# Sewer56/dxt-lossless-transform

Hardware: AMD Instinct MI355X
Metric: GiB/s BC blocks transformed (fwd+inv) (higher is better)
Workload: dtype u8

## Files before the change

### dxt-lossless-transform_amd/csrc/batch_api.cpp

```cpp
#include <hip/hip_runtime_api.h>

#include <algorithm>
#include <condition_variable>
#include <cstdlib>
#include <cstring>
#include <exception>
#include <mutex>
#include <thread>
#include <vector>

#include "../../include/dxtlt_gfx950.h"
#include "bcn_launch.h"
#include "granule_launch.h"
#include "host_common.h"

namespace {

using namespace dxtlt_host;
using dxtlt::BatchEntry;

inline uint32_t item_block_bytes(uint8_t format) { return format == 1 || format == 4 ? 8u : 16u; }

constexpr int kSlots = 4;

struct TableSlot {
    void* host = nullptr;
    void* host_mapped = nullptr;
    void* dev = nullptr;
    size_t cap = 0;
    hipEvent_t done = nullptr;
    bool pending = false;
};

struct TableRing {
    int device = -1;
    TableSlot slots[kSlots];
    int next = 0;

    ~TableRing() { release(); }
    void release()
    {
        if (device < 0)
            return;
        for (auto& s : slots) {
            if (s.host) (void)hipHostFree(s.host);
            if (s.dev) (void)hipFree(s.dev);
            if (s.done) (void)hipEventDestroy(s.done);
            s = TableSlot{};
        }
        device = -1;
        next = 0;
    }
    hipError_t acquire(size_t bytes, TableSlot** out)
    {
        int dev = 0;
        hipError_t e = hipGetDevice(&dev);
        if (e != hipSuccess)
            return e;
        if (dev != device) {
            release();
            device = dev;
        }
        TableSlot& s = slots[next];
        next = (next + 1) % kSlots;
        if (s.pending) {
            e = hipEventSynchronize(s.done);
            if (e != hipSuccess)
                return e;
            s.pending = false;
        }
        if (s.done == nullptr) {
            e = hipEventCreateWithFlags(&s.done, hipEventDisableTiming);
            if (e != hipSuccess)
                return e;
        }
        if (s.cap < bytes) {
            if (s.host) (void)hipHostFree(s.host);
            if (s.dev) (void)hipFree(s.dev);
            s.host = s.dev = nullptr;
            s.cap = 0;
            const size_t want = bytes + bytes / 2 + 4096;
            e = hipHostMalloc(&s.host, want, hipHostMallocMapped);
            if (e == hipSuccess)
                e = hipHostGetDevicePointer(&s.host_mapped, s.host, 0);
            if (e == hipSuccess)
                e = hipMalloc(&s.dev, want);
            if (e != hipSuccess)
                return e;
            s.cap = want;
        }
        *out = &s;
        return hipSuccess;
    }
};

thread_local TableRing g_ring;

const bool kTableByCopyEngine = dxtlt::experiment_env("DXTLT_BATCH_TABLE_COPY") != nullptr && dxtlt::experiment_env("DXTLT_BATCH_TABLE_COPY")[0] == '1';

hipError_t upload_table(TableSlot* slot, size_t bytes, hipStream_t stream)
{
    if (kTableByCopyEngine)
        return hipMemcpyAsync(slot->dev, slot->host, bytes, hipMemcpyHostToDevice, stream);
    return dxtlt::launch_table_upload(slot->host_mapped, slot->dev, bytes, stream);
}

}

extern "C" int32_t dxtlt_transform_batch_device(const DxtltBatchItem* items, size_t count, void* hip_stream)
{
    if (count == 0)
        return kOk;
    if (items == nullptr)
        return fail(kInvalidArgument, "NULL item array with count > 0");
    for (size_t i = 0; i < count; ++i) {
        const DxtltBatchItem& it = items[i];
        if (it.format < 1 || it.format > 7)
            return fail(kInvalidArgument, "batch item: format must be 1..5 (BC1..BC5), 6 (BC6H) or 7 (BC7; 6 and 7 are this build's "
                                          "own formats)");
        if (it.len % item_block_bytes(it.format) != 0)
            return fail(kInvalidLength, "batch item: len is not a multiple of the block size");
        if (it.decorrelation_mode > 3 && dxtlt::format_has_colour(it.format))
            return fail(kInvalidArgument, "batch item: decorrelation_mode must be 0..3");
        if (it.len > 0 && (it.d_input == nullptr || it.d_output == nullptr))
            return fail(kInvalidArgument, "batch item: NULL device buffer with len > 0");
    }
    for (const int format : {7, 6}) {
        uint64_t granules[2] = {0, 0};
        for (size_t i = 0; i < count; ++i)
            if (items[i].format == format)
                granules[items[i].inverse ? 1 : 0] += items[i].len / 16 / 1024;
        if (granules[0] > 0xFFFFFFull || granules[1] > 0xFFFFFFull)
            return fail(kInvalidArgument, dxtlt::granule::named(format, "batch too large for one launch (256 GiB or more of ", " in one direction)"));
    }
    hipStream_t user = static_cast<hipStream_t>(hip_stream);

    struct Group {
        std::vector<BatchEntry> entries;
        uint32_t wgs = 0;
        uint32_t uniform_wgs = 0;
        bool uniform = true;
    };
    constexpr int kGroups = 5 * 2 * 16;
    std::vector<Group> groups(kGroups);
    auto group_settings = [](int gi) {
        dxtlt::Settings s{};
        s.variant = (gi >> 2) & 3;
        s.split_alpha = ((gi >> 1) & 1) != 0;
        s.split_colour = (gi & 1) != 0;
        return s;
    };
    std::vector<size_t> singles;
    for (size_t i = 0; i < count; ++i) {
        const DxtltBatchItem& it = items[i];
        if (it.len == 0 || dxtlt::granule::is_granule_format(it.format))
            continue;
        if (it.len >= (size_t(64) << 30))
            return fail(kInvalidArgument, "batch item of 64 GiB or more: use the single-buffer entry point");
        const bool colour = dxtlt::format_has_colour(it.format);
        const int sa = dxtlt::format_has_alpha_split(it.format) && it.split_alpha_endpoints ? 1 : 0;
        const int sc = colour && it.split_colour_endpoints ? 1 : 0, mode = colour ? it.decorrelation_mode : 0;
        const int gi = (((it.format - 1) * 2 + (it.inverse ? 1 : 0)) << 4) | (mode << 2) | (sa << 1) | sc;
        Group& g = groups[gi];
        BatchEntry e{};
        e.src = static_cast<const uint8_t*>(it.d_input);
        e.dst = static_cast<uint8_t*>(it.d_output);
        e.blocks = it.len / item_block_bytes(it.format);
        e.first_wg = g.wgs;
        const uint32_t wgs = dxtlt::plan_batch_entry((dxtlt::Format)it.format, it.inverse != 0, group_settings(gi), e);
        if (wgs == 0xFFFFFFFFu) {
            singles.push_back(i);
            continue;
        }
        if ((uint64_t)g.wgs + wgs > 0xFFFFFFull)
            return fail(kInvalidArgument, "batch too large for one launch (64 GiB or more of one format, direction and settings)");
        g.wgs += wgs;
        g.entries.push_back(e);
        if (g.entries.size() == 1)
            g.uniform_wgs = wgs;
        else if (wgs != g.uniform_wgs)
            g.uniform = false;
    }
    static const bool no_uniform = dxtlt::experiment_env("DXTLT_BATCH_NO_UNIFORM") != nullptr;
    static const bool no_strided = dxtlt::experiment_env("DXTLT_BATCH_NO_STRIDED") != nullptr;

    using GranuleEntry = dxtlt::granule::BatchEntry;
    struct GranulePlan {
        std::vector<GranuleEntry> entries, tails;
        std::vector<uint32_t> coarse;
        uint64_t wgs = 0;
        size_t at = 0, entry_bytes = 0, tail_bytes = 0, bytes = 0;
    };
    GranulePlan granule_plans[4];
    size_t table_bytes = 0;
    for (int q = 0; q < 4; ++q) {
        GranulePlan& p = granule_plans[q];
        const int inverse = q & 1, format = q < 2 ? 7 : 6;
        for (size_t i = 0; i < count; ++i) {
            const DxtltBatchItem& it = items[i];
            if (it.format != format || it.len == 0 || (it.inverse != 0) != (inverse != 0))
                continue;
            const uint64_t blocks = it.len / 16, tail = blocks % 1024, main = blocks - tail;
            const uint8_t* src = static_cast<const uint8_t*>(it.d_input);
            uint8_t* dst = static_cast<uint8_t*>(it.d_output);
            if (main != 0) {
                p.entries.push_back({src, dst, main, (uint32_t)p.wgs, 0});
                p.wgs += main / 1024;
            }
            if (tail != 0)
                p.tails.push_back({src + main * 16, dst + main * 16, 0, 0, (uint32_t)tail});
        }
        if (p.entries.empty() && p.tails.empty())
            continue;
        p.coarse.resize(((size_t)p.wgs + 63) / 64);
        size_t cur = 0;
        for (size_t k = 0; k < p.coarse.size(); ++k) {
            while (cur + 1 < p.entries.size() && p.entries[cur + 1].first_wg <= (uint32_t)(k * 64))
                ++cur;
            p.coarse[k] = (uint32_t)cur;
        }
        p.entry_bytes = p.entries.size() * sizeof(GranuleEntry);
        p.tail_bytes = p.tails.size() * sizeof(GranuleEntry);
        p.bytes = (p.entry_bytes + p.tail_bytes + p.coarse.size() * sizeof(uint32_t) + 15) & ~(size_t)15;
        p.at = table_bytes;
        table_bytes += p.bytes;
    }

    struct Placed {
        int gi;
        size_t at, entry_bytes;
    };
    std::vector<Placed> placed;
    for (int gi = 0; gi < kGroups; ++gi) {
        const Group& g = groups[gi];
        if (g.entries.empty())
            continue;
        const size_t entry_bytes = (g.entries.size() * sizeof(BatchEntry) + 15) & ~(size_t)15;
        placed.push_back({gi, table_bytes, entry_bytes});
        table_bytes += entry_bytes + dxtlt::batch_index_bytes(g.wgs);
    }
    if (table_bytes != 0) {
        TableSlot* slot = nullptr;
        hipError_t e = g_ring.acquire(table_bytes, &slot);
        if (e != hipSuccess)
            return fail(kDevice, "batch table staging", e);
        for (const GranulePlan& p : granule_plans) {
            if (p.bytes == 0)
                continue;
            uint8_t* h = static_cast<uint8_t*>(slot->host) + p.at;
            if (p.entry_bytes) std::memcpy(h, p.entries.data(), p.entry_bytes);
            if (p.tail_bytes) std::memcpy(h + p.entry_bytes, p.tails.data(), p.tail_bytes);
            if (!p.coarse.empty()) std::memcpy(h + p.entry_bytes + p.tail_bytes, p.coarse.data(), p.coarse.size() * sizeof(uint32_t));
        }
        std::vector<bool> wide(placed.size());
        for (size_t k = 0; k < placed.size(); ++k) {
            const Group& g = groups[placed[k].gi];
            uint8_t* h = static_cast<uint8_t*>(slot->host) + placed[k].at;
            std::memcpy(h, g.entries.data(), g.entries.size() * sizeof(BatchEntry));
            wide[k] = dxtlt::build_batch_index(g.entries.data(), g.entries.size(), g.wgs, h + placed[k].entry_bytes);
        }
        e = upload_table(slot, table_bytes, user);
        const char* what = "batch table copy / launch";
        for (int q = 0; q < 4 && e == hipSuccess; ++q) {
            const GranulePlan& p = granule_plans[q];
            const int inverse = q & 1, format = q < 2 ? 7 : 6;
            if (p.bytes == 0)
                continue;
            const uint8_t* d = static_cast<const uint8_t*>(slot->dev) + p.at;
            e = dxtlt::granule::launch_batch(format, inverse != 0, reinterpret_cast<const GranuleEntry*>(d),
                                             reinterpret_cast<const uint32_t*>(d + p.entry_bytes + p.tail_bytes), (uint32_t)p.entries.size(),
                                             (uint32_t)p.wgs, reinterpret_cast<const GranuleEntry*>(d + p.entry_bytes),
                                             (uint32_t)p.tails.size(), user);
            if (e != hipSuccess)
                what = format == 7 ? "BC7 batch table copy / launch" : "BC6H batch table copy / launch";
        }
        for (size_t k = 0; k < placed.size() && e == hipSuccess; ++k) {
            const int gi = placed[k].gi;
            Group& g = groups[gi];
            const size_t n = g.entries.size();
            const bool uniform = g.uniform && !no_uniform;
            bool strided = uniform && !no_strided;
            const int64_t src_stride = n >= 2 ? (int64_t)(g.entries[1].src - g.entries[0].src) : 0;
            const int64_t dst_stride = n >= 2 ? (int64_t)(g.entries[1].dst - g.entries[0].dst) : 0;
            for (size_t i = 1; i < n && strided; ++i) {
                const BatchEntry &a = g.entries[0], &b = g.entries[i];
                strided = b.blocks == a.blocks && b.full_tiles == a.full_tiles && b.form == a.form && b.halo_vecs == a.halo_vecs &&
                          std::memcmp(b.shift, a.shift, sizeof a.shift) == 0 && std::memcmp(b.gbase, a.gbase, sizeof a.gbase) == 0 &&
                          b.src == a.src + (int64_t)i * src_stride && b.dst == a.dst + (int64_t)i * dst_stride;
            }
            const uint8_t* d = static_cast<const uint8_t*>(slot->dev) + placed[k].at;
            e = dxtlt::launch_batch((dxtlt::Format)((gi >> 5) + 1), ((gi >> 4) & 1) != 0, group_settings(gi),
                                    reinterpret_cast<const BatchEntry*>(d), d + placed[k].entry_bytes, (uint32_t)n, g.wgs,
                                    uniform ? g.uniform_wgs : 0, wide[k], user, strided ? &g.entries[0] : nullptr, src_stride, dst_stride);
        }
        hipError_t ev = hipEventRecord(slot->done, user);
        slot->pending = ev == hipSuccess;
        if (e != hipSuccess)
            return fail(kDevice, what, e);
        if (ev != hipSuccess)
            return fail(kDevice, "batch event", ev);
    }
    for (size_t i : singles) {
        const DxtltBatchItem& it = items[i];
        dxtlt::Settings s{};
        s.variant = it.decorrelation_mode;
        s.split_alpha = it.split_alpha_endpoints != 0;
        s.split_colour = it.split_colour_endpoints != 0;
        s = dxtlt::effective_settings((dxtlt::Format)it.format, s);
        const uint64_t blocks = it.len / item_block_bytes(it.format);
        const hipError_t e = dxtlt::launch_transform((dxtlt::Format)it.format, it.inverse != 0, s, it.d_input, it.d_output,
                                                     dxtlt::Range{blocks, 0, blocks}, user);
        if (e != hipSuccess)
            return fail(kDevice, "batch item launch", e);
    }
    return kOk;
}

extern "C" uint32_t dxtlt_debug_plan_batch(int32_t format, int32_t inverse, int32_t variant, int32_t split_alpha, int32_t split_colour,
                                           const uint64_t* src_addresses, const uint64_t* dst_addresses, const uint64_t* blocks, size_t count,
                                           DxtltDebugPlannedEntry* entries_out, uint8_t* index_out, size_t index_capacity,
                                           uint32_t* index_is_wide_out)
{
    if (index_is_wide_out)
        *index_is_wide_out = 0;
    if (format < 1 || format > 5 || (count != 0 && (!src_addresses || !dst_addresses || !blocks || !entries_out)))
        return 0xFFFFFFFFu;
    dxtlt::Settings s{};
    s.variant = variant;
    s.split_alpha = split_alpha != 0;
    s.split_colour = split_colour != 0;
    s = dxtlt::effective_settings((dxtlt::Format)format, s);
    std::vector<BatchEntry> entries;
    uint32_t total = 0;
    for (size_t i = 0; i < count; ++i) {
        BatchEntry e{};
        e.src = reinterpret_cast<const uint8_t*>(static_cast<uintptr_t>(src_addresses[i]));
        e.dst = reinterpret_cast<uint8_t*>(static_cast<uintptr_t>(dst_addresses[i]));
        e.blocks = blocks[i];
        e.first_wg = total;
        const uint32_t wgs = dxtlt::plan_batch_entry((dxtlt::Format)format, inverse != 0, s, e);
        if (wgs == 0xFFFFFFFFu || (uint64_t)total + wgs > 0xFFFFFFull)
            return 0xFFFFFFFFu;
        if (wgs == 0)
            e.end_wg = e.first_wg;
        total += wgs;
        DxtltDebugPlannedEntry& o = entries_out[i];
        o.first_wg = e.first_wg;
        o.end_wg = e.end_wg;
        o.full_tiles = e.full_tiles;
        o.form = e.form;
        o.halo_vecs = e.halo_vecs;
        std::memcpy(o.shift, e.shift, sizeof o.shift);
        std::memcpy(o.gbase, e.gbase, sizeof o.gbase);
        if (wgs != 0)
            entries.push_back(e);
    }
    if (total != 0) {
        if (index_out == nullptr || index_capacity < dxtlt::batch_index_bytes(total))
            return 0xFFFFFFFFu;
        const bool wide = dxtlt::build_batch_index(entries.data(), entries.size(), total, index_out);
        if (index_is_wide_out)
            *index_is_wide_out = wide ? 1 : 0;
    }
    return total;
}

// ... 353 lines not shown
```

### dxt-lossless-transform_amd/csrc/batch_kernels.hip

```cpp
#include <cstdlib>
#include <cstring>
#include <vector>

#include "bcn_device.h"

namespace dxtlt {

struct BatchView {
    const uint8_t* src;
    uint8_t* dst;
    uint64_t blocks;
    uint32_t first_wg, end_wg, full_tiles;
    uint32_t flags;
    uint32_t shifts[2];
    uint64_t gbase[6];
};

__device__ __forceinline__ BatchView load_batch_entry(const BatchEntry* entry)
{
    const uint64_t* q = reinterpret_cast<const uint64_t*>(entry);
    const uint32_t* w = reinterpret_cast<const uint32_t*>(entry);
    BatchView v;
    v.src = (const uint8_t*)(global_cptr)q[0];
    v.dst = (uint8_t*)(global_ptr)q[1];
// ... 127 lines not shown
            en = load_batch_entry(entries + e);
        }
    }
    const uint32_t n_wgs = en.end_wg - en.first_wg;
    uint32_t local = wg - en.first_wg;
    if (n_wgs >= 8) {
        local += (en.first_wg + n_wgs - 1u - e) & 7u;
        local = local >= n_wgs ? local - n_wgs : local;
    }
    const bool aligned = (en.flags & 0xFF) == kBatchAligned;
    if (aligned && local < en.full_tiles) {
        if constexpr (INVERSE)
            inv_aligned_tile<FMT, VARIANT, SA, SC, THREADS>(en.src, en.dst, en.blocks, 0, local, lds);
        else
            fwd_aligned_tile<FMT, VARIANT, SA, SC, THREADS>(en.src, en.dst, en.blocks, 0, local, lds);
        WG_TIMING_END(1);
        return;
    }
    Shifts sh;
#pragma unroll
    for (int i = 0; i < 6; ++i) {
        sh.d[i] = (int)((en.shifts[i >> 2] >> (8 * (i & 3))) & 127u);
        sh.gbase[i] = en.gbase[i];
    }
#ifdef DXTLT_EXPERIMENTS
    sh.xcd_remap = 0;
    sh.line_policy = INVERSE ? 1 : 3;
    sh.skip_partial = 0;
#endif
    sh.natural = 1;
    sh.halo_vecs = (int)(en.flags >> 8) & 0xFF;
    sh.full_tiles = en.full_tiles;
    sh.range_blocks = en.blocks;
    if constexpr (INVERSE) {
        if (local < en.full_tiles) {
            const uint64_t tile = xcd_contiguous_tile(local, en.full_tiles);
            inv_shift_tile<FMT, VARIANT, SA, SC, THREADS>(en.src, en.dst, en.blocks, 0, sh, tile, lds);
            WG_TIMING_END(2);
            return;
        }
        inv_shift_edge_tile<FMT, VARIANT, SA, SC, THREADS>(en.src, en.dst, en.blocks, sh, en.full_tiles, lds);
        WG_TIMING_END(4);
    } else {
        if (local != 0 && local < en.full_tiles) {
            fwd_halo_tile<FMT, VARIANT, SA, SC, kNormNone, true, THREADS>(en.src, en.dst, en.blocks, 0, sh, local, lds);
            WG_TIMING_END(2);
            return;
        }
        fwd_halo_edge_tile<FMT, VARIANT, SA, SC, kNormNone, true, THREADS>(en.src, en.dst, sh, local, lds);
        WG_TIMING_END(local == 0 ? 3 : 4);
    }
}

uint32_t plan_batch_entry(Format fmt, bool inverse, const Settings& s, BatchEntry& e)
{
    if (e.blocks == 0)
        return 0;
    const Settings es = effective_settings(fmt, s);
    const Streams S = make_streams(fmt, es.split_alpha, es.split_colour);
    const void* soa = inverse ? (const void*)e.src : (const void*)e.dst;
    const uint64_t T = (uint64_t)tile_blocks(fmt, batch_tile_threads(fmt, es.split_colour, inverse));
    const uint64_t tiles = e.blocks / T, rest = e.blocks % T;
    const uint64_t mask = inverse ? 15 : (uint64_t)(kHaloAlign - 1);
    bool on_lines = true, stream_tails = false;
    int d[6] = {0, 0, 0, 0, 0, 0}, halo_blocks = 0;
    for (int i = 0; i < S.n; ++i) {
        const uint64_t base = reinterpret_cast<uintptr_t>(soa) + (uint64_t)S.off[i] * e.blocks;
        d[i] = (int)(base & mask);
        on_lines = on_lines && (base & 127) == 0;
        stream_tails = stream_tails || d[i] != 0;
        halo_blocks = std::max(halo_blocks, (d[i] + S.width[i] - 1) / S.width[i]);
    }
    if (!shifts_are_natural(S, d))
        return 0xFFFFFFFFu;
    e.form = on_lines ? 1 : 0;
    e.natural = 1;
    e.reserved = 0;
    e.reserved2[0] = e.reserved2[1] = 0;
    const int per_vec = 16 / fmt_block(fmt);
    e.halo_vecs = inverse ? 0 : (uint8_t)((halo_blocks + per_vec - 1) / per_vec);
    for (int i = 0; i < 6; ++i) {
        e.shift[i] = (uint8_t)d[i];
        e.gbase[i] = i < S.n ? (uint64_t)S.off[i] * e.blocks - (uint64_t)d[i] : 0;
    }
    e.full_tiles = (uint32_t)tiles;
    const bool edge = rest != 0 || (!inverse && stream_tails);
    const uint32_t wgs = (uint32_t)tiles + (edge ? 1u : 0u);
    e.end_wg = e.first_wg + wgs;
    return wgs;
}

bool build_batch_index(const BatchEntry* entries, size_t n_entries, uint32_t total_wgs, uint8_t* index)
{
    const size_t n_base = batch_index_base_count(total_wgs), n_delta = batch_index_delta_count(total_wgs);
    uint32_t* base = reinterpret_cast<uint32_t*>(index);
    std::memset(index, 0, batch_index_bytes(total_wgs));
    std::vector<uint32_t> d(n_delta);
    uint32_t largest = 0;
    size_t cur = 0;
    for (size_t j = 0; j < n_delta; ++j) {
        const uint32_t wg = (uint32_t)(j * kBatchIndexWgs);
        while (cur + 1 < n_entries && entries[cur].end_wg <= wg)
            ++cur;
        if (wg % kBatchBaseWgs == 0)
            base[wg / kBatchBaseWgs] = (uint32_t)cur;
        d[j] = (uint32_t)(cur - base[wg / kBatchBaseWgs]);
        largest = std::max(largest, d[j]);
    }
    const bool wide = largest > 255;
    uint8_t* delta = index + n_base * 4;
    for (size_t j = 0; j < n_delta; ++j) {
        if (wide) {
            delta[2 * j] = (uint8_t)d[j];
            delta[2 * j + 1] = (uint8_t)(d[j] >> 8);
        } else {
            delta[j] = (uint8_t)d[j];
        }
    }
    return wide;
}

namespace {

using BatchFn = void (*)(const BatchEntry*, const uint8_t*, uint32_t, uint32_t, uint32_t, StridedBatch);

template <int FMT, int VARIANT, bool SA, bool SC>
BatchFn batch_fn(bool inverse) { return inverse ? batch_kernel<FMT, VARIANT, SA, SC, true> : batch_kernel<FMT, VARIANT, SA, SC, false>; }

template <int FMT, int VARIANT>
BatchFn batch_splits(bool sa, bool sc, bool inverse)
{
    if constexpr (FMT == kBc3) {
        if (sa)
            return sc ? batch_fn<FMT, VARIANT, true, true>(inverse) : batch_fn<FMT, VARIANT, true, false>(inverse);
    }
    return sc ? batch_fn<FMT, VARIANT, false, true>(inverse) : batch_fn<FMT, VARIANT, false, false>(inverse);
}

template <int FMT>
BatchFn batch_bc45(bool split_endpoints, bool inverse)
{
    return split_endpoints ? batch_fn<FMT, kNone, true, false>(inverse) : batch_fn<FMT, kNone, false, false>(inverse);
}

template <int FMT>
BatchFn batch_variant(int variant, bool sa, bool sc, bool inverse)
{
    switch (variant) {
    case kNone: return batch_splits<FMT, kNone>(sa, sc, inverse);
    case kVar1: return batch_splits<FMT, kVar1>(sa, sc, inverse);
    case kVar2: return batch_splits<FMT, kVar2>(sa, sc, inverse);
    default: return batch_splits<FMT, kVar3>(sa, sc, inverse);
    }
}

}

hipError_t launch_batch(Format fmt, bool inverse, const Settings& s, const BatchEntry* d_entries, const uint8_t* d_index,
                        uint32_t n_entries, uint32_t total_wgs, uint32_t uniform_wgs, bool wide_index, hipStream_t stream,
                        const BatchEntry* strided_first, int64_t src_stride, int64_t dst_stride)
{
    if (n_entries == 0 || total_wgs == 0)
        return hipSuccess;
    if (s.variant < 0 || s.variant > 3 || total_wgs > 0xFFFFFFu)
        return hipErrorInvalidValue;
    if (uniform_wgs != 0 && (uint64_t)uniform_wgs * n_entries != total_wgs)
        return hipErrorInvalidValue;
    const uint32_t magic = uniform_wgs > 1 ? (uint32_t)((1ull << 32) / uniform_wgs) : uniform_wgs == 1 ? 0xFFFFFFFFu : n_entries;
    static const bool no_array = experiment_env("DXTLT_BATCH_NO_ARRAY") != nullptr;
    if (strided_first != nullptr && uniform_wgs != 0 && !no_array && strided_first->form == 1) {
        const hipError_t e = launch_tiled_array(fmt, inverse, s, strided_first->src, strided_first->dst, strided_first->blocks, n_entries,
// ... 29 lines not shown
```

### dxt-lossless-transform_amd/csrc/bcn_launch.h

```cpp
#pragma once
#include <hip/hip_runtime_api.h>
#include <stddef.h>
#include <stdint.h>

#include <cstdlib>

namespace dxtlt {

inline const char* experiment_env(const char* name)
{
#ifdef DXTLT_EXPERIMENTS
    return std::getenv(name);
#else
    (void)name;
    return nullptr;
#endif
}

enum Format : int { kBc1 = 1, kBc2 = 2, kBc3 = 3, kBc4 = 4, kBc5 = 5 };

struct Settings {
    int variant;
    bool split_alpha;
    bool split_colour;
// ... 106 lines not shown
    if (!format_has_colour(f)) {
        e.variant = 0;
        e.split_colour = false;
    }
    return e;
}

struct Streams {
    int n;
    int width[6];
    int off[6];
};

constexpr Streams make_streams(int fmt, bool split_alpha, bool split_colour)
{
    Streams s{};
    int n = 0, off = 0;
    if (fmt == kBc4 || fmt == kBc5) {
        for (int h = 0; h < (fmt == kBc5 ? 2 : 1); ++h) {
            if (split_alpha) {
                s.width[n] = 1; s.off[n] = off; off += 1; ++n;
                s.width[n] = 1; s.off[n] = off; off += 1; ++n;
            } else {
                s.width[n] = 2; s.off[n] = off; off += 2; ++n;
            }
            s.width[n] = 6; s.off[n] = off; off += 6; ++n;
        }
        s.n = n;
        return s;
    }
    if (fmt == kBc3) {
        if (split_alpha) {
            s.width[n] = 1; s.off[n] = off; off += 1; ++n;
            s.width[n] = 1; s.off[n] = off; off += 1; ++n;
        } else {
            s.width[n] = 2; s.off[n] = off; off += 2; ++n;
        }
        s.width[n] = 6; s.off[n] = off; off += 6; ++n;
    }
    if (fmt == kBc2) {
        s.width[n] = 8; s.off[n] = off; off += 8; ++n;
    }
    if (split_colour) {
        s.width[n] = 2; s.off[n] = off; off += 2; ++n;
        s.width[n] = 2; s.off[n] = off; off += 2; ++n;
    } else {
        s.width[n] = 4; s.off[n] = off; off += 4; ++n;
    }
    s.width[n] = 4; s.off[n] = off; off += 4; ++n;
    s.n = n;
    return s;
}

}
```

### include/dxtlt_gfx950.h

```cpp
#ifndef DXTLT_GFX950_H
#define DXTLT_GFX950_H

#include <stdbool.h>
#include <stddef.h>
#include <stdint.h>

#include "dlt_size_estimator.h"

#ifdef __cplusplus
extern "C" {
#endif

#define DXTLT_OK 0
#define DXTLT_E_INVALID_LENGTH 1
#define DXTLT_E_INVALID_ARGUMENT 2
#define DXTLT_E_NO_DEVICE 3
#define DXTLT_E_DEVICE 4
#define DXTLT_E_ESTIMATOR 5
#define DXTLT_E_ALLOCATION 6

#define DXTLT_YCOCG_NONE 0
#define DXTLT_YCOCG_VARIANT1 1
#define DXTLT_YCOCG_VARIANT2 2
#define DXTLT_YCOCG_VARIANT3 3
// ... 29 lines not shown
void dxtlt_set_auto_estimator_threads(int32_t threads);
int32_t dxtlt_get_auto_estimator_threads(void);
int32_t dxtlt_set_auto_estimator_threads_for_this_thread(int32_t cap);

int32_t dxtlt_transform_bc1_with_settings_device(const void *d_input, void *d_output, size_t len,
                                                 uint8_t decorrelation_mode, bool split_colour_endpoints,
                                                 void *hip_stream);
int32_t dxtlt_untransform_bc1_with_settings_device(const void *d_input, void *d_output, size_t len,
                                                   uint8_t decorrelation_mode, bool split_colour_endpoints,
                                                   void *hip_stream);
int32_t dxtlt_transform_bc2_with_settings_device(const void *d_input, void *d_output, size_t len,
                                                 uint8_t decorrelation_mode, bool split_colour_endpoints,
                                                 void *hip_stream);
int32_t dxtlt_untransform_bc2_with_settings_device(const void *d_input, void *d_output, size_t len,
                                                   uint8_t decorrelation_mode, bool split_colour_endpoints,
                                                   void *hip_stream);
int32_t dxtlt_transform_bc3_with_settings_device(const void *d_input, void *d_output, size_t len,
                                                 uint8_t decorrelation_mode, bool split_alpha_endpoints,
                                                 bool split_colour_endpoints, void *hip_stream);
int32_t dxtlt_untransform_bc3_with_settings_device(const void *d_input, void *d_output, size_t len,
                                                   uint8_t decorrelation_mode, bool split_alpha_endpoints,
                                                   bool split_colour_endpoints, void *hip_stream);

int32_t dxtlt_transform_range_device(int32_t format, bool inverse, const void *d_src, void *d_dst,
                                     uint64_t total_blocks, uint64_t first_block, uint64_t num_blocks,
                                     uint8_t decorrelation_mode, bool split_alpha_endpoints,
                                     bool split_colour_endpoints, void *hip_stream);

typedef struct DxtltBatchItem {
    const void *d_input;
    void *d_output;
    uint64_t len;
    uint8_t format;
    uint8_t inverse;
    uint8_t decorrelation_mode;
    uint8_t split_alpha_endpoints;
    uint8_t split_colour_endpoints;
    uint8_t reserved[3];
} DxtltBatchItem;
int32_t dxtlt_transform_batch_device(const DxtltBatchItem *items, size_t count, void *hip_stream);
typedef struct DxtltDebugPlannedEntry {
    uint32_t first_wg, end_wg;
    uint32_t full_tiles;
    uint8_t form;
    uint8_t halo_vecs;
    uint8_t shift[6];
    uint64_t gbase[6];
} DxtltDebugPlannedEntry;
uint32_t dxtlt_debug_plan_batch(int32_t format, int32_t inverse, int32_t variant, int32_t split_alpha, int32_t split_colour,
                                const uint64_t *src_addresses, const uint64_t *dst_addresses, const uint64_t *blocks, size_t count,
                                DxtltDebugPlannedEntry *entries_out, uint8_t *index_out, size_t index_capacity,
                                uint32_t *index_is_wide_out);

typedef struct DxtltDebugPlannedLaunch {
    int32_t kind;
    int32_t threads;
    uint32_t workgroups;
    uint32_t full_tiles;
    uint64_t range_blocks;
    uint64_t aos_offset;
    uint8_t shift[6];
    uint8_t halo_vecs;
    uint8_t natural;
    uint64_t gbase[6];
} DxtltDebugPlannedLaunch;
int32_t dxtlt_debug_plan_transform(int32_t format, int32_t inverse, int32_t variant, int32_t split_alpha, int32_t split_colour,
                                   uint64_t src_address, uint64_t dst_address, uint64_t total_blocks, uint64_t first_block,
                                   uint64_t num_blocks, DxtltDebugPlannedLaunch *out, int32_t cap);

int32_t dxtlt_transform_batch_host(const DxtltBatchItem *items, size_t count);

int32_t dxtlt_transform_sharded(int32_t format, bool inverse, const uint8_t *input_ptr, uint8_t *output_ptr,
                                size_t len, uint8_t decorrelation_mode, bool split_alpha_endpoints,
                                bool split_colour_endpoints, int32_t num_devices);

typedef struct DxtltShardStat {
    int32_t device;
    int32_t cpus_bound;
    uint64_t first_block;
    uint64_t blocks;
    double seconds;
} DxtltShardStat;
int32_t dxtlt_sharded_last_stats(DxtltShardStat *out, int32_t cap);

int32_t dxtlt_pci_local_cpulist(const char *pci_bdf, char *out, size_t cap);
int32_t dxtlt_device_local_cpulist(int32_t device, char *out, size_t cap);
int32_t dxtlt_bind_thread_to_cpulist(const char *cpulist);

int32_t dxtlt_fill_splitmix64_device(void *d_dst, size_t len_bytes, uint64_t seed, uint64_t first_qword,
                                     void *hip_stream);
const char *dxtlt_last_error(void);
int32_t dxtlt_device_count(void);
size_t dxtlt_host_route_threshold_bytes(void);
void dxtlt_set_host_route_threshold_bytes(size_t bytes);
void dxtlt_set_tuning(int32_t tile_threads, int32_t force_path);
int32_t dxtlt_tuning_mask(void);
const char *dxtlt_version(void);
void dxtlt_release_thread_resources(void);

#ifdef __cplusplus
}
#endif
#endif
```

Measured before the change: 3191.

## Restructure batch planning into count and place passes, skip tables for regular groups

Batch planning is split into a counting pass that builds a per-group context once and reuses the workgroup count for entries with matching size and alignment, plus a staging pass that writes entries straight into pinned host memory. Groups whose items are evenly strided with identical plans skip the per-entry table and index upload entirely and go down an array-style launch. The index builder also writes deltas in place instead of using a temporary vector. The intent is to cut host-side per-call planning, allocation and table upload costs for large batches, at the price of more complex two-pass logic that has to stay consistent between the passes.

```diff
diff --git a/dxt-lossless-transform_amd/csrc/batch_api.cpp b/dxt-lossless-transform_amd/csrc/batch_api.cpp
--- a/dxt-lossless-transform_amd/csrc/batch_api.cpp
+++ b/dxt-lossless-transform_amd/csrc/batch_api.cpp
@@ -2,6 +2,7 @@
 
 #include <algorithm>
 #include <condition_variable>
+#include <cstdio>
 #include <cstdlib>
 #include <cstring>
 #include <exception>
@@ -105,14 +106,74 @@
     return dxtlt::launch_table_upload(slot->host_mapped, slot->dev, bytes, stream);
 }
 
-}
-
-extern "C" int32_t dxtlt_transform_batch_device(const DxtltBatchItem* items, size_t count, void* hip_stream)
-{
-    if (count == 0)
-        return kOk;
-    if (items == nullptr)
-        return fail(kInvalidArgument, "NULL item array with count > 0");
+constexpr int kGroups = 5 * 2 * 16;
+
+inline dxtlt::Settings group_settings(int gi)
+{
+    dxtlt::Settings s{};
+    s.variant = (gi >> 2) & 3;
+    s.split_alpha = ((gi >> 1) & 1) != 0;
+    s.split_colour = (gi & 1) != 0;
+    return s;
+}
+
+inline int group_of(const DxtltBatchItem& it)
+{
+    const bool colour = dxtlt::format_has_colour(it.format);
+    const int sa = dxtlt::format_has_alpha_split(it.format) && it.split_alpha_endpoints ? 1 : 0;
+    const int sc = colour && it.split_colour_endpoints ? 1 : 0, mode = colour ? it.decorrelation_mode : 0;
+    return (((it.format - 1) * 2 + (it.inverse ? 1 : 0)) << 4) | (mode << 2) | (sa << 1) | sc;
+}
+
+inline uint64_t address_of(const void* p) { return static_cast<uint64_t>(reinterpret_cast<uintptr_t>(p)); }
+
+struct GroupPlan {
+    int gi = 0;
+    dxtlt::BatchGroupContext ctx{};
+    uint32_t count = 0;
+    uint32_t wgs = 0;
+    uint32_t uniform_wgs = 0;
+    bool uniform = true;
+    bool regular = true;
+    bool has_table = false;
+    bool wide = false;
+    uint64_t src0 = 0, dst0 = 0, blocks0 = 0;
+    int64_t src_stride = 0, dst_stride = 0;
+    BatchEntry first{};
+    size_t at = 0, entry_bytes = 0, index_bytes = 0;
+    uint32_t placed = 0, next_wg = 0;
+};
+
+using GranuleEntry = dxtlt::granule::BatchEntry;
+struct GranulePlan {
+    std::vector<GranuleEntry> entries, tails;
+    std::vector<uint32_t> coarse;
+    uint64_t wgs = 0;
+    size_t at = 0, entry_bytes = 0, tail_bytes = 0, bytes = 0;
+};
+
+struct BatchCallPlan {
+    std::vector<GroupPlan> groups;
+    int16_t slot_of[kGroups];
+    GranulePlan granule[4];
+    std::vector<size_t> singles;
+    size_t table_bytes = 0;
+};
+
+const bool kNoUniform = dxtlt::experiment_env("DXTLT_BATCH_NO_UNIFORM") != nullptr;
+const bool kNoStrided = dxtlt::experiment_env("DXTLT_BATCH_NO_STRIDED") != nullptr;
+const bool kNoArray = dxtlt::experiment_env("DXTLT_BATCH_NO_ARRAY") != nullptr;
+
+inline bool same_plan(const BatchEntry& a, const BatchEntry& b)
+{
+    return b.blocks == a.blocks && b.end_wg - b.first_wg == a.end_wg - a.first_wg && b.full_tiles == a.full_tiles && b.form == a.form &&
+           b.halo_vecs == a.halo_vecs && std::memcmp(b.shift, a.shift, sizeof a.shift) == 0 && std::memcmp(b.gbase, a.gbase, sizeof a.gbase) == 0;
+}
+
+int32_t plan_batch_call(const DxtltBatchItem* items, size_t count, BatchCallPlan& plan)
+{
+    uint64_t granules[4] = {0, 0, 0, 0};
+    size_t granule_items = 0;
     for (size_t i = 0; i < count; ++i) {
         const DxtltBatchItem& it = items[i];
         if (it.format < 1 || it.format > 7)
@@ -124,77 +185,70 @@
             return fail(kInvalidArgument, "batch item: decorrelation_mode must be 0..3");
         if (it.len > 0 && (it.d_input == nullptr || it.d_output == nullptr))
             return fail(kInvalidArgument, "batch item: NULL device buffer with len > 0");
-    }
-    for (const int format : {7, 6}) {
-        uint64_t granules[2] = {0, 0};
-        for (size_t i = 0; i < count; ++i)
-            if (items[i].format == format)
-                granules[items[i].inverse ? 1 : 0] += items[i].len / 16 / 1024;
-        if (granules[0] > 0xFFFFFFull || granules[1] > 0xFFFFFFull)
-            return fail(kInvalidArgument, dxtlt::granule::named(format, "batch too large for one launch (256 GiB or more of ", " in one direction)"));
-    }
-    hipStream_t user = static_cast<hipStream_t>(hip_stream);
-
-    struct Group {
-        std::vector<BatchEntry> entries;
-        uint32_t wgs = 0;
-        uint32_t uniform_wgs = 0;
-        bool uniform = true;
-    };
-    constexpr int kGroups = 5 * 2 * 16;
-    std::vector<Group> groups(kGroups);
-    auto group_settings = [](int gi) {
-        dxtlt::Settings s{};
-        s.variant = (gi >> 2) & 3;
-        s.split_alpha = ((gi >> 1) & 1) != 0;
-        s.split_colour = (gi & 1) != 0;
-        return s;
-    };
-    std::vector<size_t> singles;
+        if (dxtlt::granule::is_granule_format(it.format) && it.len != 0) {
+            granules[(it.format == 7 ? 0 : 2) + (it.inverse ? 1 : 0)] += it.len / 16 / 1024;
+            ++granule_items;
+        }
+    }
+    for (int q = 0; q < 4; ++q)
+        if (granules[q] > 0xFFFFFFull)
+            return fail(kInvalidArgument, dxtlt::granule::named(q < 2 ? 7 : 6, "batch too large for one launch (256 GiB or more of ", " in one direction)"));
+
+    std::memset(plan.slot_of, 0xFF, sizeof plan.slot_of);
     for (size_t i = 0; i < count; ++i) {
         const DxtltBatchItem& it = items[i];
         if (it.len == 0 || dxtlt::granule::is_granule_format(it.format))
             continue;
         if (it.len >= (size_t(64) << 30))
             return fail(kInvalidArgument, "batch item of 64 GiB or more: use the single-buffer entry point");
-        const bool colour = dxtlt::format_has_colour(it.format);
-        const int sa = dxtlt::format_has_alpha_split(it.format) && it.split_alpha_endpoints ? 1 : 0;
-        const int sc = colour && it.split_colour_endpoints ? 1 : 0, mode = colour ? it.decorrelation_mode : 0;
-        const int gi = (((it.format - 1) * 2 + (it.inverse ? 1 : 0)) << 4) | (mode << 2) | (sa << 1) | sc;
-        Group& g = groups[gi];
-        BatchEntry e{};
-        e.src = static_cast<const uint8_t*>(it.d_input);
-        e.dst = static_cast<uint8_t*>(it.d_output);
-        e.blocks = it.len / item_block_bytes(it.format);
-        e.first_wg = g.wgs;
-        const uint32_t wgs = dxtlt::plan_batch_entry((dxtlt::Format)it.format, it.inverse != 0, group_settings(gi), e);
+        const int gi = group_of(it);
+        if (plan.slot_of[gi] < 0) {
+            plan.slot_of[gi] = (int16_t)plan.groups.size();
+            plan.groups.emplace_back();
+            plan.groups.back().gi = gi;
+            plan.groups.back().ctx = dxtlt::make_batch_group((dxtlt::Format)it.format, it.inverse != 0, group_settings(gi));
+        }
+        GroupPlan& g = plan.groups[(size_t)plan.slot_of[gi]];
+        const uint64_t src = address_of(it.d_input), dst = address_of(it.d_output), blocks = it.len / item_block_bytes(it.format);
+        const uint64_t soa = it.inverse ? src : dst;
+        const uint32_t wgs = g.count != 0 && blocks == g.blocks0 && ((soa ^ (it.inverse ? g.src0 : g.dst0)) & 127) == 0
+                                 ? g.uniform_wgs : dxtlt::count_batch_entry(g.ctx, soa, blocks);
         if (wgs == 0xFFFFFFFFu) {
-            singles.push_back(i);
-            continue;
-        }
-        if ((uint64_t)g.wgs + wgs > 0xFFFFFFull)
-            return fail(kInvalidArgument, "batch too large for one launch (64 GiB or more of one format, direction and settings)");
+            plan.singles.push_back(i);
+            continue;
+        }
+        if ((uint64_t)g.wgs + wgs > 0xFFFFFFull) {
+            thread_local char text[160];
+            std::snprintf(text, sizeof text, "batch too large for one launch (more than 2^24 tiles of %d KiB of one format, direction and settings)",
+                          g.ctx.threads * 16 / 1024);
+            return fail(kInvalidArgument, text);
+        }
+        if (g.count == 0) {
+            g.src0 = src;
+            g.dst0 = dst;
+            g.blocks0 = blocks;
+            g.uniform_wgs = wgs;
+        } else {
+            if (g.count == 1) {
+                g.src_stride = (int64_t)(src - g.src0);
+                g.dst_stride = (int64_t)(dst - g.dst0);
+            }
+            g.uniform = g.uniform && wgs == g.uniform_wgs;
+            g.regular = g.regular && blocks == g.blocks0 && src == g.src0 + (uint64_t)g.count * (uint64_t)g.src_stride &&
+                        dst == g.dst0 + (uint64_t)g.count * (uint64_t)g.dst_stride;
+        }
         g.wgs += wgs;
-        g.entries.push_back(e);
-        if (g.entries.size() == 1)
-            g.uniform_wgs = wgs;
-        else if (wgs != g.uniform_wgs)
-            g.uniform = false;
-    }
-    static const bool no_uniform = dxtlt::experiment_env("DXTLT_BATCH_NO_UNIFORM") != nullptr;
-    static const bool no_strided = dxtlt::experiment_env("DXTLT_BATCH_NO_STRIDED") != nullptr;
-
-    using GranuleEntry = dxtlt::granule::BatchEntry;
-    struct GranulePlan {
-        std::vector<GranuleEntry> entries, tails;
-        std::vector<uint32_t> coarse;
-        uint64_t wgs = 0;
-        size_t at = 0, entry_bytes = 0, tail_bytes = 0, bytes = 0;
-    };
-    GranulePlan granule_plans[4];
-    size_t table_bytes = 0;
-    for (int q = 0; q < 4; ++q) {
-        GranulePlan& p = granule_plans[q];
+        ++g.count;
+    }
+    plan.groups.erase(std::remove_if(plan.groups.begin(), plan.groups.end(), [](const GroupPlan& g) { return g.count == 0; }), plan.groups.end());
+    std::sort(plan.groups.begin(), plan.groups.end(), [](const GroupPlan& a, const GroupPlan& b) { return a.gi < b.gi; });
+    std::memset(plan.slot_of, 0xFF, sizeof plan.slot_of);
+    for (size_t k = 0; k < plan.groups.size(); ++k)
+        plan.slot_of[plan.groups[k].gi] = (int16_t)k;
+
+    plan.table_bytes = 0;
+    for (int q = 0; q < 4 && granule_items != 0; ++q) {
+        GranulePlan& p = plan.granule[q];
         const int inverse = q & 1, format = q < 2 ? 7 : 6;
         for (size_t i = 0; i < count; ++i) {
             const DxtltBatchItem& it = items[i];
@@ -222,85 +276,139 @@
         p.entry_bytes = p.entries.size() * sizeof(GranuleEntry);
         p.tail_bytes = p.tails.size() * sizeof(GranuleEntry);
         p.bytes = (p.entry_bytes + p.tail_bytes + p.coarse.size() * sizeof(uint32_t) + 15) & ~(size_t)15;
-        p.at = table_bytes;
-        table_bytes += p.bytes;
-    }
-
-    struct Placed {
-        int gi;
-        size_t at, entry_bytes;
-    };
-    std::vector<Placed> placed;
-    for (int gi = 0; gi < kGroups; ++gi) {
-        const Group& g = groups[gi];
-        if (g.entries.empty())
-            continue;
-        const size_t entry_bytes = (g.entries.size() * sizeof(BatchEntry) + 15) & ~(size_t)15;
-        placed.push_back({gi, table_bytes, entry_bytes});
-        table_bytes += entry_bytes + dxtlt::batch_index_bytes(g.wgs);
-    }
-    if (table_bytes != 0) {
-        TableSlot* slot = nullptr;
-        hipError_t e = g_ring.acquire(table_bytes, &slot);
+        p.at = plan.table_bytes;
+        plan.table_bytes += p.bytes;
+    }
+
+    for (GroupPlan& g : plan.groups) {
+        g.first.src = reinterpret_cast<const uint8_t*>(static_cast<uintptr_t>(g.src0));
+        g.first.dst = reinterpret_cast<uint8_t*>(static_cast<uintptr_t>(g.dst0));
+        g.first.blocks = g.blocks0;
+        g.first.first_wg = 0;
+        (void)dxtlt::plan_batch_entry(g.ctx, g.first);
+        g.uniform = g.uniform && !kNoUniform;
+        g.regular = g.regular && g.uniform && !kNoStrided;
+        const int64_t soa_stride = g.ctx.inverse ? g.src_stride : g.dst_stride;
+        if (g.regular && g.count >= 2 && (soa_stride & 127) != 0) {
+            const uint32_t low = (uint32_t)(soa_stride & 127), period = 128u / (low & (0u - low));
+            for (uint32_t i = 1; i < period && i < g.count && g.regular; ++i) {
+                BatchEntry e{};
+                e.src = reinterpret_cast<const uint8_t*>(static_cast<uintptr_t>(g.src0 + (uint64_t)i * (uint64_t)g.src_stride));
+                e.dst = reinterpret_cast<uint8_t*>(static_cast<uintptr_t>(g.dst0 + (uint64_t)i * (uint64_t)g.dst_stride));
+                e.blocks = g.blocks0;
+                g.regular = dxtlt::plan_batch_entry(g.ctx, e) != 0xFFFFFFFFu && same_plan(g.first, e);
+            }
+        }
+        g.has_table = !g.regular || kNoArray;
+        if (g.has_table) {
+            g.entry_bytes = ((size_t)g.count * sizeof(BatchEntry) + 15) & ~(size_t)15;
+            g.index_bytes = dxtlt::batch_index_bytes(g.wgs);
+            g.at = plan.table_bytes;
+            plan.table_bytes += g.entry_bytes + g.index_bytes;
+        }
+    }
+    return kOk;
+}
+
+int32_t stage_batch_call(const DxtltBatchItem* items, size_t count, BatchCallPlan& plan, uint8_t* host)
+{
+    for (const GranulePlan& p : plan.granule) {
+        if (p.bytes == 0)
+            continue;
+        uint8_t* h = host + p.at;
+        if (p.entry_bytes) std::memcpy(h, p.entries.data(), p.entry_bytes);
+        if (p.tail_bytes) std::memcpy(h + p.entry_bytes, p.tails.data(), p.tail_bytes);
+        if (!p.coarse.empty()) std::memcpy(h + p.entry_bytes + p.tail_bytes, p.coarse.data(), p.coarse.size() * sizeof(uint32_t));
+    }
+    bool any = false;
+    for (const GroupPlan& g : plan.groups)
+        any = any || g.has_table;
+    if (!any)
+        return kOk;
+    for (size_t i = 0; i < count; ++i) {
+        const DxtltBatchItem& it = items[i];
+        if (it.len == 0 || dxtlt::granule::is_granule_format(it.format))
+            continue;
+        const int slot = plan.slot_of[group_of(it)];
+        if (slot < 0 || !plan.groups[(size_t)slot].has_table)
+            continue;
+        GroupPlan& g = plan.groups[(size_t)slot];
+        BatchEntry e{};
+        e.src = static_cast<const uint8_t*>(it.d_input);
+        e.dst = static_cast<uint8_t*>(it.d_output);
+        e.blocks = it.len / item_block_bytes(it.format);
+        e.first_wg = g.next_wg;
+        const uint32_t wgs = dxtlt::plan_batch_entry(g.ctx, e);
+        if (wgs == 0xFFFFFFFFu)
+            continue;
+        if (g.placed >= g.count || (uint64_t)g.next_wg + wgs > g.wgs)
+            return fail(kDevice, "batch table: the placing pass disagrees with the count pass");
+        reinterpret_cast<BatchEntry*>(host + g.at)[g.placed++] = e;
+        g.next_wg += wgs;
+    }
+    for (GroupPlan& g : plan.groups) {
+        if (!g.has_table)
+            continue;
+        if (g.placed != g.count || g.next_wg != g.wgs)
+            return fail(kDevice, "batch table: the placing pass disagrees with the count pass");
+        g.wide = dxtlt::build_batch_index(reinterpret_cast<const BatchEntry*>(host + g.at), g.count, g.wgs, host + g.at + g.entry_bytes);
+    }
+    return kOk;
+}
+
+}
+
+extern "C" int32_t dxtlt_transform_batch_device(const DxtltBatchItem* items, size_t count, void* hip_stream)
+{
+    if (count == 0)
+        return kOk;
+    if (items == nullptr)
+        return fail(kInvalidArgument, "NULL item array with count > 0");
+    BatchCallPlan plan;
+    if (const int32_t rc = plan_batch_call(items, count, plan); rc != kOk)
+        return rc;
+    hipStream_t user = static_cast<hipStream_t>(hip_stream);
+
+    TableSlot* slot = nullptr;
+    hipError_t e = hipSuccess;
+    const char* what = "batch table copy / launch";
+    if (plan.table_bytes != 0) {
+        e = g_ring.acquire(plan.table_bytes, &slot);
         if (e != hipSuccess)
             return fail(kDevice, "batch table staging", e);
-        for (const GranulePlan& p : granule_plans) {
-            if (p.bytes == 0)
-                continue;
-            uint8_t* h = static_cast<uint8_t*>(slot->host) + p.at;
-            if (p.entry_bytes) std::memcpy(h, p.entries.data(), p.entry_bytes);
-            if (p.tail_bytes) std::memcpy(h + p.entry_bytes, p.tails.data(), p.tail_bytes);
-            if (!p.coarse.empty()) std::memcpy(h + p.entry_bytes + p.tail_bytes, p.coarse.data(), p.coarse.size() * sizeof(uint32_t));
-        }
-        std::vector<bool> wide(placed.size());
-        for (size_t k = 0; k < placed.size(); ++k) {
-            const Group& g = groups[placed[k].gi];
-            uint8_t* h = static_cast<uint8_t*>(slot->host) + placed[k].at;
-            std::memcpy(h, g.entries.data(), g.entries.size() * sizeof(BatchEntry));
-            wide[k] = dxtlt::build_batch_index(g.entries.data(), g.entries.size(), g.wgs, h + placed[k].entry_bytes);
-        }
-        e = upload_table(slot, table_bytes, user);
-        const char* what = "batch table copy / launch";
-        for (int q = 0; q < 4 && e == hipSuccess; ++q) {
-            const GranulePlan& p = granule_plans[q];
-            const int inverse = q & 1, format = q < 2 ? 7 : 6;
-            if (p.bytes == 0)
-                continue;
-            const uint8_t* d = static_cast<const uint8_t*>(slot->dev) + p.at;
-            e = dxtlt::granule::launch_batch(format, inverse != 0, reinterpret_cast<const GranuleEntry*>(d),
-                                             reinterpret_cast<const uint32_t*>(d + p.entry_bytes + p.tail_bytes), (uint32_t)p.entries.size(),
-                                             (uint32_t)p.wgs, reinterpret_cast<const GranuleEntry*>(d + p.entry_bytes),
-                                             (uint32_t)p.tails.size(), user);
-            if (e != hipSuccess)
-                what = format == 7 ? "BC7 batch table copy / launch" : "BC6H batch table copy / launch";
-        }
-        for (size_t k = 0; k < placed.size() && e == hipSuccess; ++k) {
-            const int gi = placed[k].gi;
-            Group& g = groups[gi];
-            const size_t n = g.entries.size();
-            const bool uniform = g.uniform && !no_uniform;
-            bool strided = uniform && !no_strided;
-            const int64_t src_stride = n >= 2 ? (int64_t)(g.entries[1].src - g.entries[0].src) : 0;
-            const int64_t dst_stride = n >= 2 ? (int64_t)(g.entries[1].dst - g.entries[0].dst) : 0;
-            for (size_t i = 1; i < n && strided; ++i) {
-                const BatchEntry &a = g.entries[0], &b = g.entries[i];
-                strided = b.blocks == a.blocks && b.full_tiles == a.full_tiles && b.form == a.form && b.halo_vecs == a.halo_vecs &&
-                          std::memcmp(b.shift, a.shift, sizeof a.shift) == 0 && std::memcmp(b.gbase, a.gbase, sizeof a.gbase) == 0 &&
-                          b.src == a.src + (int64_t)i * src_stride && b.dst == a.dst + (int64_t)i * dst_stride;
-            }
-            const uint8_t* d = static_cast<const uint8_t*>(slot->dev) + placed[k].at;
-            e = dxtlt::launch_batch((dxtlt::Format)((gi >> 5) + 1), ((gi >> 4) & 1) != 0, group_settings(gi),
-                                    reinterpret_cast<const BatchEntry*>(d), d + placed[k].entry_bytes, (uint32_t)n, g.wgs,
-                                    uniform ? g.uniform_wgs : 0, wide[k], user, strided ? &g.entries[0] : nullptr, src_stride, dst_stride);
-        }
-        hipError_t ev = hipEventRecord(slot->done, user);
+        if (const int32_t rc = stage_batch_call(items, count, plan, static_cast<uint8_t*>(slot->host)); rc != kOk)
+            return rc;
+        e = upload_table(slot, plan.table_bytes, user);
+    }
+    for (int q = 0; q < 4 && e == hipSuccess; ++q) {
+        const GranulePlan& p = plan.granule[q];
+        const int inverse = q & 1, format = q < 2 ? 7 : 6;
+        if (p.bytes == 0)
+            continue;
+        const uint8_t* d = static_cast<const uint8_t*>(slot->dev) + p.at;
+        e = dxtlt::granule::launch_batch(format, inverse != 0, reinterpret_cast<const GranuleEntry*>(d),
+                                         reinterpret_cast<const uint32_t*>(d + p.entry_bytes + p.tail_bytes), (uint32_t)p.entries.size(),
+                                         (uint32_t)p.wgs, reinterpret_cast<const GranuleEntry*>(d + p.entry_bytes),
+                                         (uint32_t)p.tails.size(), user);
+        if (e != hipSuccess)
+            what = format == 7 ? "BC7 batch table copy / launch" : "BC6H batch table copy / launch";
+    }
+    for (size_t k = 0; k < plan.groups.size() && e == hipSuccess; ++k) {
+        const GroupPlan& g = plan.groups[k];
+        const uint8_t* d = g.has_table ? static_cast<const uint8_t*>(slot->dev) + g.at : nullptr;
+        e = dxtlt::launch_batch((dxtlt::Format)((g.gi >> 5) + 1), ((g.gi >> 4) & 1) != 0, group_settings(g.gi),
+                                reinterpret_cast<const BatchEntry*>(d), g.has_table ? d + g.entry_bytes : nullptr, g.count, g.wgs,
+                                g.uniform ? g.uniform_wgs : 0, g.wide, user, g.regular ? &g.first : nullptr, g.src_stride, g.dst_stride);
+    }
+    if (slot != nullptr) {
+        const hipError_t ev = hipEventRecord(slot->done, user);
         slot->pending = ev == hipSuccess;
-        if (e != hipSuccess)
-            return fail(kDevice, what, e);
-        if (ev != hipSuccess)
+        if (e == hipSuccess && ev != hipSuccess)
             return fail(kDevice, "batch event", ev);
     }
-    for (size_t i : singles) {
+    if (e != hipSuccess)
+        return fail(kDevice, what, e);
+    for (size_t i : plan.singles) {
         const DxtltBatchItem& it = items[i];
         dxtlt::Settings s{};
         s.variant = it.decorrelation_mode;
@@ -308,10 +416,55 @@
         s.split_colour = it.split_colour_endpoints != 0;
         s = dxtlt::effective_settings((dxtlt::Format)it.format, s);
         const uint64_t blocks = it.len / item_block_bytes(it.format);
-        const hipError_t e = dxtlt::launch_transform((dxtlt::Format)it.format, it.inverse != 0, s, it.d_input, it.d_output,
-                                                     dxtlt::Range{blocks, 0, blocks}, user);
+        e = dxtlt::launch_transform((dxtlt::Format)it.format, it.inverse != 0, s, it.d_input, it.d_output,
+                                    dxtlt::Range{blocks, 0, blocks}, user);
         if (e != hipSuccess)
             return fail(kDevice, "batch item launch", e);
+    }
+    return kOk;
+}
+
+extern "C" int32_t dxtlt_debug_plan_batch_call(const DxtltBatchItem* items, size_t count, void* staging, size_t staging_capacity,
+                                               DxtltDebugBatchCallReport* report, DxtltDebugBatchCallGroup* groups_out, size_t groups_capacity)
+{
+    if (report == nullptr || (count != 0 && items == nullptr) || (groups_capacity != 0 && groups_out == nullptr))
+        return fail(kInvalidArgument, "dxtlt_debug_plan_batch_call: NULL argument");
+    *report = DxtltDebugBatchCallReport{};
+    BatchCallPlan plan;
+    if (const int32_t rc = plan_batch_call(items, count, plan); rc != kOk)
+        return rc;
+    report->table_bytes = plan.table_bytes;
+    report->groups = (uint32_t)plan.groups.size();
+    report->singles = (uint32_t)plan.singles.size();
+    for (int q = 0; q < 4; ++q) {
+        report->granule_table_offset[q] = plan.granule[q].at;
+        report->granule_table_bytes[q] = plan.granule[q].bytes;
+    }
+    if (staging != nullptr) {
+        if (staging_capacity < plan.table_bytes || (reinterpret_cast<uintptr_t>(staging) & 15) != 0)
+            return fail(kInvalidArgument, "dxtlt_debug_plan_batch_call: the staging buffer is too small or not 16-byte aligned");
+        if (const int32_t rc = stage_batch_call(items, count, plan, static_cast<uint8_t*>(staging)); rc != kOk)
+            return rc;
+        report->staged = 1;
+    }
+    for (size_t k = 0; k < plan.groups.size() && k < groups_capacity; ++k) {
+        const GroupPlan& g = plan.groups[k];
+        const dxtlt::Settings s = group_settings(g.gi);
+        DxtltDebugBatchCallGroup& o = groups_out[k];
+        o = DxtltDebugBatchCallGroup{};
+        o.format = (uint8_t)((g.gi >> 5) + 1);
+        o.inverse = (uint8_t)((g.gi >> 4) & 1);
+        o.decorrelation_mode = (uint8_t)s.variant;
+        o.split_alpha_endpoints = s.split_alpha ? 1 : 0;
+        o.split_colour_endpoints = s.split_colour ? 1 : 0;
+        o.regular = g.regular ? 1 : 0;
+        o.wide_index = g.wide ? 1 : 0;
+        o.uniform = g.uniform ? 1 : 0;
+        o.entries = g.count;
+        o.workgroups = g.wgs;
+        o.table_offset = g.has_table ? g.at : 0;
+        o.entry_bytes = g.has_table ? g.entry_bytes : 0;
+        o.table_bytes = g.has_table ? g.entry_bytes + g.index_bytes : 0;
     }
     return kOk;
 }
diff --git a/dxt-lossless-transform_amd/csrc/batch_kernels.hip b/dxt-lossless-transform_amd/csrc/batch_kernels.hip
--- a/dxt-lossless-transform_amd/csrc/batch_kernels.hip
+++ b/dxt-lossless-transform_amd/csrc/batch_kernels.hip
@@ -203,50 +203,96 @@
     }
 }
 
-uint32_t plan_batch_entry(Format fmt, bool inverse, const Settings& s, BatchEntry& e)
+BatchGroupContext make_batch_group(Format fmt, bool inverse, const Settings& s)
+{
+    const Settings es = effective_settings(fmt, s);
+    BatchGroupContext g{};
+    g.fmt = fmt;
+    g.inverse = inverse;
+    g.threads = batch_tile_threads(fmt, es.split_colour, inverse);
+    g.tile_blocks = (uint64_t)tile_blocks(fmt, g.threads);
+    g.shift_mask = inverse ? 15 : (uint64_t)(kHaloAlign - 1);
+    g.vec_blocks = 16 / fmt_block(fmt);
+    g.streams = make_streams(fmt, es.split_alpha, es.split_colour);
+    return g;
+}
+
+namespace {
+
+inline bool batch_entry_shifts(const BatchGroupContext& g, uint64_t soa, uint64_t blocks, int (&d)[6], bool& on_lines, bool& stream_tails)
+{
+    const Streams& S = g.streams;
+    on_lines = true;
+    stream_tails = false;
+    for (int i = 0; i < 6; ++i)
+        d[i] = 0;
+    for (int i = 0; i < S.n; ++i) {
+        const uint64_t base = soa + (uint64_t)S.off[i] * blocks;
+        d[i] = (int)(base & g.shift_mask);
+        on_lines = on_lines && (base & 127) == 0;
+        stream_tails = stream_tails || d[i] != 0;
+    }
+    return shifts_are_natural(S, d) != 0;
+}
+
+inline uint32_t batch_entry_wgs(const BatchGroupContext& g, uint64_t blocks, bool stream_tails)
+{
+    const uint64_t tiles = blocks / g.tile_blocks, rest = blocks % g.tile_blocks;
+    const bool edge = rest != 0 || (!g.inverse && stream_tails);
+    return (uint32_t)tiles + (edge ? 1u : 0u);
+}
+
+}
+
+uint32_t count_batch_entry(const BatchGroupContext& g, uint64_t soa_address, uint64_t blocks)
+{
+    if (blocks == 0)
+        return 0;
+    int d[6];
+    bool on_lines, stream_tails;
+    if (!batch_entry_shifts(g, soa_address, blocks, d, on_lines, stream_tails))
+        return 0xFFFFFFFFu;
+    return batch_entry_wgs(g, blocks, stream_tails);
+}
+
+uint32_t plan_batch_entry(const BatchGroupContext& g, BatchEntry& e)
 {
     if (e.blocks == 0)
         return 0;
-    const Settings es = effective_settings(fmt, s);
-    const Streams S = make_streams(fmt, es.split_alpha, es.split_colour);
-    const void* soa = inverse ? (const void*)e.src : (const void*)e.dst;
-    const uint64_t T = (uint64_t)tile_blocks(fmt, batch_tile_threads(fmt, es.split_colour, inverse));
-    const uint64_t tiles = e.blocks / T, rest = e.blocks % T;
-    const uint64_t mask = inverse ? 15 : (uint64_t)(kHaloAlign - 1);
-    bool on_lines = true, stream_tails = false;
-    int d[6] = {0, 0, 0, 0, 0, 0}, halo_blocks = 0;
-    for (int i = 0; i < S.n; ++i) {
-        const uint64_t base = reinterpret_cast<uintptr_t>(soa) + (uint64_t)S.off[i] * e.blocks;
-        d[i] = (int)(base & mask);
-        on_lines = on_lines && (base & 127) == 0;
-        stream_tails = stream_tails || d[i] != 0;
+    const Streams& S = g.streams;
+    const void* soa = g.inverse ? (const void*)e.src : (const void*)e.dst;
+    int d[6];
+    bool on_lines, stream_tails;
+    if (!batch_entry_shifts(g, reinterpret_cast<uintptr_t>(soa), e.blocks, d, on_lines, stream_tails))
+        return 0xFFFFFFFFu;
+    int halo_blocks = 0;
+    for (int i = 0; i < S.n; ++i)
         halo_blocks = std::max(halo_blocks, (d[i] + S.width[i] - 1) / S.width[i]);
-    }
-    if (!shifts_are_natural(S, d))
-        return 0xFFFFFFFFu;
     e.form = on_lines ? 1 : 0;
     e.natural = 1;
     e.reserved = 0;
     e.reserved2[0] = e.reserved2[1] = 0;
-    const int per_vec = 16 / fmt_block(fmt);
-    e.halo_vecs = inverse ? 0 : (uint8_t)((halo_blocks + per_vec - 1) / per_vec);
+    e.halo_vecs = g.inverse ? 0 : (uint8_t)((halo_blocks + g.vec_blocks - 1) / g.vec_blocks);
     for (int i = 0; i < 6; ++i) {
         e.shift[i] = (uint8_t)d[i];
         e.gbase[i] = i < S.n ? (uint64_t)S.off[i] * e.blocks - (uint64_t)d[i] : 0;
     }
-    e.full_tiles = (uint32_t)tiles;
-    const bool edge = rest != 0 || (!inverse && stream_tails);
-    const uint32_t wgs = (uint32_t)tiles + (edge ? 1u : 0u);
+    e.full_tiles = (uint32_t)(e.blocks / g.tile_blocks);
+    const uint32_t wgs = batch_entry_wgs(g, e.blocks, stream_tails);
     e.end_wg = e.first_wg + wgs;
     return wgs;
 }
 
+uint32_t plan_batch_entry(Format fmt, bool inverse, const Settings& s, BatchEntry& e)
+{
+    return plan_batch_entry(make_batch_group(fmt, inverse, s), e);
+}
+
 bool build_batch_index(const BatchEntry* entries, size_t n_entries, uint32_t total_wgs, uint8_t* index)
 {
     const size_t n_base = batch_index_base_count(total_wgs), n_delta = batch_index_delta_count(total_wgs);
     uint32_t* base = reinterpret_cast<uint32_t*>(index);
-    std::memset(index, 0, batch_index_bytes(total_wgs));
-    std::vector<uint32_t> d(n_delta);
+    uint8_t* delta = index + n_base * 4;
     uint32_t largest = 0;
     size_t cur = 0;
     for (size_t j = 0; j < n_delta; ++j) {
@@ -255,19 +301,20 @@
             ++cur;
         if (wg % kBatchBaseWgs == 0)
             base[wg / kBatchBaseWgs] = (uint32_t)cur;
-        d[j] = (uint32_t)(cur - base[wg / kBatchBaseWgs]);
-        largest = std::max(largest, d[j]);
+        const uint32_t d = (uint32_t)(cur - base[wg / kBatchBaseWgs]);
+        largest = std::max(largest, d);
+        delta[2 * j] = (uint8_t)d;
+        delta[2 * j + 1] = (uint8_t)(d >> 8);
     }
     const bool wide = largest > 255;
-    uint8_t* delta = index + n_base * 4;
-    for (size_t j = 0; j < n_delta; ++j) {
-        if (wide) {
-            delta[2 * j] = (uint8_t)d[j];
-            delta[2 * j + 1] = (uint8_t)(d[j] >> 8);
-        } else {
-            delta[j] = (uint8_t)d[j];
-        }
-    }
+    size_t used = 2 * n_delta;
+    if (!wide) {
+        for (size_t j = 0; j < n_delta; ++j)
+            delta[j] = delta[2 * j];
+        used = n_delta;
+    }
+    const size_t end = batch_index_bytes(total_wgs) - n_base * 4;
+    std::memset(delta + used, 0, end - used);
     return wide;
 }
 
diff --git a/dxt-lossless-transform_amd/csrc/bcn_launch.h b/dxt-lossless-transform_amd/csrc/bcn_launch.h
--- a/dxt-lossless-transform_amd/csrc/bcn_launch.h
+++ b/dxt-lossless-transform_amd/csrc/bcn_launch.h
@@ -182,4 +182,17 @@
     return s;
 }
 
+struct BatchGroupContext {
+    Format fmt;
+    bool inverse;
+    int threads;
+    uint64_t tile_blocks;
+    uint64_t shift_mask;
+    int vec_blocks;
+    Streams streams;
+};
+BatchGroupContext make_batch_group(Format fmt, bool inverse, const Settings& s);
+uint32_t plan_batch_entry(const BatchGroupContext& g, BatchEntry& e);
+uint32_t count_batch_entry(const BatchGroupContext& g, uint64_t soa_address, uint64_t blocks);
+
 }
diff --git a/include/dxtlt_gfx950.h b/include/dxtlt_gfx950.h
--- a/include/dxtlt_gfx950.h
+++ b/include/dxtlt_gfx950.h
@@ -105,6 +105,24 @@
                                 DxtltDebugPlannedEntry *entries_out, uint8_t *index_out, size_t index_capacity,
                                 uint32_t *index_is_wide_out);
 
+typedef struct DxtltDebugBatchCallGroup {
+    uint8_t format, inverse, decorrelation_mode, split_alpha_endpoints, split_colour_endpoints;
+    uint8_t regular;
+    uint8_t uniform;
+    uint8_t wide_index;
+    uint32_t entries, workgroups;
+    uint64_t table_offset, entry_bytes, table_bytes;
+} DxtltDebugBatchCallGroup;
+typedef struct DxtltDebugBatchCallReport {
+    uint64_t table_bytes;
+    uint64_t granule_table_offset[4], granule_table_bytes[4];
+    uint32_t groups, singles;
+    uint32_t staged;
+    uint32_t reserved;
+} DxtltDebugBatchCallReport;
+int32_t dxtlt_debug_plan_batch_call(const DxtltBatchItem *items, size_t count, void *staging, size_t staging_capacity,
+                                    DxtltDebugBatchCallReport *report, DxtltDebugBatchCallGroup *groups_out, size_t groups_capacity);
+
 typedef struct DxtltDebugPlannedLaunch {
     int32_t kind;
     int32_t threads;
```

Measured after the change: 3190. About the same (-0.0%).
